# gchq/annchor

Measured on AMD Instinct MI355X. Metric: knn_graph_builds_per_s (1 / Annchor.fit() wall-clock; BASELINE: k-NN graph build time + recall@k), higher is better.
Workload: dtype int32 bit-vectors (Levenshtein) + f64 (bounds/regression/selection); 1 GPU; load_strings Levenshtein N=1600 n_anchors=15 k=25 p_work=0.12 niters=2; parallelism=one GPU

## Files before the change

### annchor_amd/csrc/common.h

```cpp
#pragma once
#include <hip/hip_runtime.h>

#include <cstdint>
#include <cstdio>
#include <cstring>
#include <string>
#include <vector>
#include <chrono>

#include "../../include/annchor_hip.h"

#define ANN_WAVE 64

struct DevBuf {
    void *p = nullptr;
    size_t cap = 0;
    bool in_arena = false;
    template <typename T> T *as() const { return reinterpret_cast<T *>(p); }
};

struct ProfEntry {
    const char *name;
    double ms = 0;
    int64_t launches = 0;
    double alg_bytes = 0;
};

struct PendingEvent {
    int entry;
    hipEvent_t a, b;
};

struct annchor_ctx {
    int device = 0;
    hipStream_t stream = nullptr;
    std::string err;
    hipDeviceProp_t prop;

    char *arena = nullptr;
    size_t arena_size = 0, arena_off = 0;

    int metric = ANNCHOR_METRIC_NONE;
    int64_t nx = 0;
    DevBuf sym, soff, slen;
    int alphabet = 0, maxlen = 0;
    bool sym_wide = false;
    int lev_gl0 = 0;
    double lev_frac0 = 0.0;
    DevBuf lev_order;
    int lev_nshort = 0;
    DevBuf lev_ap;
    DevBuf lev_ap_min;
    uint32_t lev_ap_epoch = 0;
    uint32_t lev_ap_probe_epoch = 0;
    DevBuf lev_cursors;
    int lev_cursor_epoch = 0;
    DevBuf lev_perm;
    DevBuf pts;
    int dim = 0;
    DevBuf hist, cost, supp;
    DevBuf hs_bin, hs_val, hs_cnt;
    int nbins = 0, max_support = 0;
    double cost_max = 0.0;
    int emd_epoch = 0;
    bool cost_is_metric = false;
    bool hist_integral = false;
    bool hist_fits_i16 = false;

    std::vector<unsigned char> model_cache;
    bool model_cache_valid = false;
    size_t model_cache_errs = 0;

    bool park_refine = false;
    hipEvent_t dl_ev = nullptr;

    uint32_t idle_gen_seed = 0;
    int64_t idle_gen_n = 0, idle_gen_done = 0, idle_gen_chunk = 0;

    void *comm = nullptr;
    int comm_world = 1, comm_rank = 0;
    void *comm_side = nullptr;
    hipStream_t comm_side_stream = nullptr;
    hipEvent_t comm_side_ev = nullptr, comm_main_ev = nullptr;
    bool comm_side_pending = false;
    double comm_timeout_s = 300.0;
    bool comm_aborted = false;
    void *comm_watch = nullptr;

    int na = 0, nA = 0;
    DevBuf Dt;
    DevBuf A;
    DevBuf anchorRank;
    DevBuf runmin, redval, redidx;

    DevBuf sid, cA, thr;
    int sid_nw = 1;
    DevBuf sidl, sidm;
    int sid_L = 0;
    DevBuf Kbits, Kpref;
    DevBuf deg, low, rowstart;
    DevBuf Iptr, Iidx;
    int64_t n = 0;
    DevBuf ij;
    bool have_bitmap = false;
    DevBuf colT, colM;

    DevBuf lb, ub, dad, RA, prob;
    DevBuf anc, ncm, label;
    bool have_features = false, have_RA = false;
    int64_t n_unc = -1;
    int64_t n_unc_after_features = -1;

    DevBuf spos, sy;
    DevBuf draw_J, draw_next, draw_q1;
    DevBuf sfeat, spred;
    DevBuf model;
    DevBuf ols_scratch;
    std::vector<DevBuf *> own_allocs;
    int prof_group_entry = -1;
    bool model_fitted = false;
    bool errs_on_device = false;
    int model_nb = 0;
    DevBuf dev_flags;
    bool dev_flags_clean = false;
    bool gn_err_clean = false;
    bool state_prewarmed = false;
    DevBuf sstats;
    DevBuf hs_key, hs_pos, hs_misc;
    int64_t nsamp = 0;

    DevBuf thresh;
    DevBuf cand, next;
    int64_t ncand = 0, nnext = 0;
    bool cand_marked = false;
    DevBuf gl_val, gl_pos, gl_cnt, gl_ncomp, marked, markcount;
    DevBuf gn_state;
    bool sel_prepared = false;
    int sel_k = 0, sel_nmin = 0;
    bool gn_pending = false;
    int gn_round = 0, gn_L = 0;
    DevBuf sel_hist, sel_state, blk_cnt, blk_off;
    DevBuf sel_pass_state;
    DevBuf tie_lists, tie_hist;
    const void *tie_hist_clean = nullptr;
    DevBuf sel2, sel_bufA, sel_bufB, sel_seg;
    const void *sel2_clean = nullptr;
    DevBuf errs, errptr;
    DevBuf ecdf_index;
    DevBuf cptr, cidx, cval;
    DevBuf c16, cbnd;
    DevBuf tmp0, tmp1, tmp2, tmp3;
    DevBuf scan_tmp;

    DevBuf stage_in, stage_out;

    bool prof_on = false;
    int prof_mode = 0;
    std::vector<hipEvent_t> ev_pool;
    std::vector<ProfEntry> prof;
    std::vector<PendingEvent> pending;
    hipEvent_t call_a = nullptr, call_b = nullptr;
    bool call_timed = false;
    static constexpr int PIN_SLOTS = 8;
    static constexpr size_t PIN_SLOT_BYTES = 64 * 1024;
    static constexpr size_t PIN_DL_BYTES = 1024 * 1024;
    static constexpr size_t PIN_TAIL_BYTES = 64;
    unsigned char *pin = nullptr;
    hipEvent_t pin_ev[PIN_SLOTS] = {};
    bool pin_busy[PIN_SLOTS] = {};
    int pin_next = 0;
};

const char *ann_set_err(annchor_ctx *c, const char *fmt, ...);

#define ANN_CHECK_HIP(c, expr)                                                                  \
    do {                                                                                        \
        hipError_t _e = (expr);                                                                 \
        if (_e != hipSuccess) {                                                                 \
            ann_set_err((c), "%s:%d: %s failed: %s", __FILE__, __LINE__, #expr,                 \
                        hipGetErrorString(_e));                                                 \
            return ANNCHOR_EHIP;                                                                \
        }                                                                                       \
    } while (0)

#define ANN_TRY(expr)                \
    do {                             \
        int _r = (expr);             \
        if (_r != ANNCHOR_OK) return _r; \
    } while (0)

#define ANN_REQUIRE(c, cond, code, ...)    \
    do {                                   \
        if (!(cond)) {                     \
            ann_set_err((c), __VA_ARGS__); \
            return (code);                 \
        }                                  \
    } while (0)

int ann_reserve(annchor_ctx *c, DevBuf &b, size_t bytes);
int ann_arena_init(annchor_ctx *c, int64_t nx);
int ann_prewarm_state(annchor_ctx *c);
void ann_lev_ap_probe(annchor_ctx *c);
size_t ann_sel2_table_bytes();
size_t ann_tie_hist_bytes();
size_t ann_sel_state_bytes();
int ann_h2d(annchor_ctx *c, void *dst, const void *src, size_t bytes);
hipError_t ann_sync(annchor_ctx *c, const char *where);
int ann_dev_alloc(annchor_ctx *c, void **p, size_t want, size_t *got);
void ann_dev_free(annchor_ctx *c, void *p, size_t bytes);
struct Sel2Epilogue;
int ann_kth_async(annchor_ctx *c, const double *vals, const uint8_t *flag, int64_t n, const int64_t *ks, int nk,
                  const unsigned long long **d_prefix, const int **d_unfinished, const Sel2Epilogue *epi = nullptr);
void ann_kth_async_done(annchor_ctx *c);
int ann_d2h(annchor_ctx *c, void *dst, const void *src, size_t bytes);
int ann_d2h_then(annchor_ctx *c, void *dst, const void *src, size_t bytes, int (*then)(annchor_ctx *));
int ann_d2h2(annchor_ctx *c, void *dst1, const void *src1, size_t bytes1, void *dst2, const void *src2, size_t bytes2);

int ann_prof_entry(annchor_ctx *c, const char *name);
struct ProfGroup {
    annchor_ctx *c;
    int entry = -1;
    hipEvent_t a = nullptr, b = nullptr;
    ProfGroup(annchor_ctx *ctx, const char *name);
    ~ProfGroup();
};

struct ProfScope {
    annchor_ctx *c;
    int entry = -1;
    hipEvent_t a = nullptr, b = nullptr;
    ProfScope(annchor_ctx *ctx, const char *name, double alg_bytes = 0);
    ~ProfScope();
};

static inline int ann_blocks(int64_t n, int per_block) { return (int)((n + per_block - 1) / per_block); }

__device__ __forceinline__ uint64_t ann_key_asc(double v)
{
    uint64_t u = (uint64_t)__double_as_longlong(v);
    return (u & 0x8000000000000000ull) ? ~u : (u | 0x8000000000000000ull);
}
__device__ __forceinline__ double ann_key_asc_inv(uint64_t k)
{
    uint64_t u = (k & 0x8000000000000000ull) ? (k & 0x7fffffffffffffffull) : ~k;
    return __longlong_as_double((long long)u);
}

template <typename T> __device__ __forceinline__ T ann_ldc(const T *__restrict__ p, int64_t t, int64_t n)
{
    return p[t < n ? t : n - 1];
}

#define ANN_STREAM_MIN_PAIRS (8ll << 20)
template <typename T> __device__ __forceinline__ void ann_store(T *p, T v, bool stream)
{
    if (stream) __builtin_nontemporal_store(v, p);
    else *p = v;
}
template <typename T> __device__ __forceinline__ T ann_load(const T *p, bool stream)
{
    return stream ? __builtin_nontemporal_load(p) : *p;
}

#define MAXBINS 64
struct RegModel {
    double e[MAXBINS + 1];
    double w[MAXBINS][3];
    double c[MAXBINS];
    int nb;
};
struct DeviceModel {
    RegModel reg;
    int32_t status[MAXBINS];
    int32_t err_status;
    int64_t rows[MAXBINS];
    int64_t errptr[MAXBINS + 1];
};

struct PairSource {
    const int2 *ij = nullptr;
    const int32_t *idx = nullptr;
    const int32_t *anchor = nullptr;
    int64_t n = 0;
    const double *pick_row = nullptr;
    double *pick_runmin = nullptr;
    int32_t *pick_out = nullptr;
    int pick_reset = 0;
    bool *pick_fused = nullptr;
};

#define ANN_MASK_ANCHORS 256
#define ANN_MAX_ANCHORS 1024
static_assert(ANN_MAX_ANCHORS < 0xffff, "wide sets list anchor ids as uint16, 0xffff pads");
static inline bool ann_sid_wide(int na) { return na > ANN_MASK_ANCHORS; }
__device__ __forceinline__ int sidm_common(const uint16_t *__restrict__ sidl, const uint64_t *__restrict__ sidm, int L, int na, int kw,
                                           int64_t i, int64_t w)
{
    const int lane = threadIdx.x & 63;
    int c = 0;
    for (int r = 0; r < L; ++r) {
        const int64_t e = i * L + r;
        const uint32_t pr = reinterpret_cast<const uint32_t *>(sidl)[e >> 1];
        const int a = __builtin_amdgcn_readfirstlane((int)((pr >> ((e & 1) * 16)) & 0xffffu));
        if (a >= na) continue;
        const uint64_t m = sidm[(size_t)a * kw + w];
        c += (int)((m >> lane) & 1ull);
    }
    return c;
}
template <int LC>
__device__ __forceinline__ int sidm_common_l(const uint16_t *__restrict__ sidl, const uint64_t *__restrict__ sidm, int na, int kw,
                                             int64_t i, int64_t w)
{
    const int lane = threadIdx.x & 63;
    int a[LC];
#pragma unroll
    for (int r = 0; r < LC; ++r) {
        const int64_t e = i * LC + r;
        const uint32_t pr = reinterpret_cast<const uint32_t *>(sidl)[e >> 1];
        a[r] = __builtin_amdgcn_readfirstlane((int)((pr >> ((e & 1) * 16)) & 0xffffu));
    }
    int c = 0;
#pragma unroll
    for (int r = 0; r < LC; ++r) {
        const uint64_t m = sidm[(size_t)(a[r] < na ? a[r] : 0) * kw + w];
        c += a[r] < na ? (int)((m >> lane) & 1ull) : 0;
    }
    return c;
}
template <int NW> struct Sid { uint64_t w[NW]; };
template <int NW> __device__ __forceinline__ Sid<NW> sid_ld(const uint64_t *__restrict__ sid, int64_t i)
{
    Sid<NW> s;
#pragma unroll
    for (int w = 0; w < NW; ++w) s.w[w] = sid[i * NW + w];
    return s;
}
template <int NW> __device__ __forceinline__ Sid<NW> sid_zero()
{
    Sid<NW> s;
#pragma unroll
    for (int w = 0; w < NW; ++w) s.w[w] = 0ull;
    return s;
}
template <int NW> __device__ __forceinline__ int sid_common(const Sid<NW> &a, const Sid<NW> &b)
{
    int c = 0;
#pragma unroll
    for (int w = 0; w < NW; ++w) c += __popcll(a.w[w] & b.w[w]);
    return c;
}
static inline int ann_sid_words(int na) { return na <= 64 ? 1 : na <= 128 ? 2 : na <= ANN_MASK_ANCHORS ? 4 : (na + 63) / 64; }
#define ANN_SID_DISPATCH(nw, CALL) do { if ((nw) == 1) { CALL(1); } else if ((nw) == 2) { CALL(2); } else if ((nw) == 4) { CALL(4); } \
                                        else { ANN_REQUIRE(c, false, ANNCHOR_ESTATE, "no mask kernel for %d-word anchor sets", (int)(nw)); } } while (0)

__device__ __forceinline__ void argmax_combine(double &v, int &i, double ov, int oi)
{
    if (ov > v || (ov == v && oi < i)) { v = ov; i = oi; }
}
int ann_metric_launch(annchor_ctx *c, const PairSource &src, double *d_out, double *d_RA, uint8_t *d_ncm);
int ann_lev_launch(annchor_ctx *c, const PairSource &src, double *d_out, double *d_RA, uint8_t *d_ncm);
int ann_lev_anchor_rounds(annchor_ctx *c, int32_t na, int32_t first, bool *done);
int ann_legacy_generate_upto(uint32_t seed, int64_t ndraws, int64_t upto);
static inline long long ann_now_ns()
{
    return (long long)std::chrono::duration_cast<std::chrono::nanoseconds>(std::chrono::steady_clock::now().time_since_epoch()).count();
}
int ann_legacy_scan(uint32_t seed, const int64_t *counts, const int64_t *want, int32_t nbins, uint32_t *J, const int64_t *joff,
                    void (*after_bin)(int, void *), void *user, unsigned long long *progress = nullptr);
int ann_model_prefetch_begin(annchor_ctx *c, unsigned char *at, size_t room, size_t *used);
void ann_model_prefetch_end(annchor_ctx *c, const unsigned char *at, size_t used);
int ann_euclid_launch(annchor_ctx *c, const PairSource &src, double *d_out, double *d_RA, uint8_t *d_ncm);
int ann_emd_launch(annchor_ctx *c, const PairSource &src, double *d_out, double *d_RA, uint8_t *d_ncm);

int ann_exclusive_scan_i32_to_i64(annchor_ctx *c, const int32_t *in, int64_t *out, int64_t n);
int ann_kth_smallest(annchor_ctx *c, const double *vals, const uint8_t *flag, int64_t n, const int64_t *ks,
                     int nk, double *h_out);

int ann_set_anchor_flags(annchor_ctx *c, const int64_t *hA, int nA);
int ann_dev_flags(annchor_ctx *c);
int ann_predict_merge_device(annchor_ctx *c, const RegModel *d_model, int first_iteration, int is_metric);
```

### annchor_amd/csrc/refine.hip

```cpp
#include "common.h"
#include "rowsel.h"

__global__ __launch_bounds__(ROW_THREADS) void k_comp_count(const int64_t *__restrict__ Iptr, RowSrc src, int32_t *__restrict__ cnt)
{
    __shared__ uint32_t acc;
    if (threadIdx.x == 0) acc = 0;
    __syncthreads();
    const int64_t i = row_of_block(gridDim.x), b = Iptr[i];
    const int len = (int)(Iptr[i + 1] - b);
    const RowView rv = row_view(src, i, b);
    uint32_t s = 0;
    for (int k0 = threadIdx.x; k0 < len; k0 += 4 * ROW_THREADS) {
        bool u[4];
#pragma unroll
        for (int e = 0; e < 4; ++e) u[e] = rv.unc(min(k0 + e * ROW_THREADS, len - 1));
#pragma unroll
        for (int e = 0; e < 4; ++e) s += (k0 + e * ROW_THREADS < len) && !u[e];
    }
    if (s) atomicAdd(&acc, s);
    __syncthreads();
    if (threadIdx.x == 0) cnt[i] = (int32_t)acc;
}

__global__ __launch_bounds__(ROW_THREADS) void k_comp_fill(const int64_t *__restrict__ Iptr, RowSrc src, const int2 *__restrict__ ij,
                                                          const int64_t *__restrict__ cptr,
                                                          int32_t *__restrict__ cidx, double *__restrict__ cval)
{
    __shared__ uint32_t wsum[ROW_THREADS / 64];
    const int64_t i = row_of_block(gridDim.x), b = Iptr[i];
    const int len = (int)(Iptr[i + 1] - b);
    const RowView rv = row_view(src, i, b);
    const int32_t *Iidx = src.Iidx;
    const double *RA = src.RA;
    int64_t w = cptr[i];
    for (int base = 0; base < len; base += ROW_THREADS) {
        const int k = base + threadIdx.x;
        uint32_t f = 0;
        if (k < len) f = !rv.unc(k);
        uint32_t tot;
        const uint32_t ex = row_block_scan(f, wsum, &tot);
        if (f) {
            const int32_t p = Iidx[b + k];
            const int2 q = ij[p];
            cidx[w + ex] = q.x == (int)i ? q.y : q.x;
            cval[w + ex] = RA[p];
        }
        w += tot;
        __syncthreads();
    }
}

__device__ __forceinline__ uint32_t comp_zero_bytes(uint4 v) { return 16u - (uint32_t)(__popc(v.x) + __popc(v.y) + __popc(v.z) + __popc(v.w)); }
#define COMP_ONES make_uint4(0x01010101u, 0x01010101u, 0x01010101u, 0x01010101u)

__global__ __launch_bounds__(ROW_THREADS) void k_comp_count_direct(const int64_t *__restrict__ Iptr, RowSrc src, int32_t *__restrict__ cnt)
{
    __shared__ uint32_t acc;
    if (threadIdx.x == 0) acc = 0;
    __syncthreads();
    const int64_t i = row_of_block(gridDim.x), b = Iptr[i];
    const int len = (int)(Iptr[i + 1] - b);
    const RowView rv = row_view(src, i, b);
    const int nA = min(rv.low, len);
    uint32_t s = 0;
    for (int part = 0; part < 2; ++part) {
        const uint8_t *p = part ? rv.ncm : rv.Tm;
        const int n = part ? len - nA : nA;
        const int head = min(n, (int)((16u - (uint32_t)(reinterpret_cast<uintptr_t>(p) & 15u)) & 15u));
        if ((int)threadIdx.x < head) s += p[threadIdx.x] == 0;
        const uint4 *q = reinterpret_cast<const uint4 *>(p + head);
        const int n16 = (n - head) >> 4;
        for (int t = threadIdx.x; t < n16; t += ROW_THREADS) s += comp_zero_bytes(q[t]);
        for (int k = head + (n16 << 4) + threadIdx.x; k < n; k += ROW_THREADS) s += p[k] == 0;
    }
#pragma unroll
    for (int off = 32; off > 0; off >>= 1) s += __shfl_xor(s, off);
    if ((threadIdx.x & 63) == 0 && s) atomicAdd(&acc, s);
    __syncthreads();
    if (threadIdx.x == 0) cnt[i] = (int32_t)acc;
}

__global__ __launch_bounds__(ROW_THREADS) void k_comp_fill_direct(const int64_t *__restrict__ Iptr, RowSrc src, const int2 *__restrict__ ij,
                                                                 const int64_t *__restrict__ cptr,
                                                                 int32_t *__restrict__ cidx, double *__restrict__ cval)
{
    __shared__ uint32_t wsum[ROW_THREADS / 64];
    const int64_t i = row_of_block(gridDim.x), b = Iptr[i];
    const int len = (int)(Iptr[i + 1] - b);
    const RowView rv = row_view(src, i, b);
    const int32_t *Iidx = src.Iidx + b;
    const double *RA = src.RA;
    const int nA = min(rv.low, len);
    int64_t w = cptr[i];
    auto step = [&](uint4 v, int k0) {
        const uint32_t z = comp_zero_bytes(v);
        uint32_t tot;
        uint32_t ex = row_block_scan(z, wsum, &tot);
        if (z) {
            const uint32_t wd[4] = {v.x, v.y, v.z, v.w};
#pragma unroll
            for (int e = 0; e < 16; ++e)
                if (((wd[e >> 2] >> (8 * (e & 3))) & 0xFFu) == 0u) {
                    const int32_t p = Iidx[k0 + e];
                    const int2 q = ij[p];
                    cidx[w + ex] = q.x == (int)i ? q.y : q.x;
                    cval[w + ex] = RA[p];
                    ++ex;
                }
        }
        w += tot;
        __syncthreads();
    };
    for (int part = 0; part < 2; ++part) {
        const uint8_t *p = part ? rv.ncm : rv.Tm;
        const int n = part ? len - nA : nA, kofs = part ? nA : 0;
        const int head = min(n, (int)((16u - (uint32_t)(reinterpret_cast<uintptr_t>(p) & 15u)) & 15u));
        if (head) {
            uint4 v = COMP_ONES;
            if ((int)threadIdx.x < head) v.x = 0x01010100u | p[threadIdx.x];
            step(v, kofs + (int)threadIdx.x);
        }
        const uint4 *q = reinterpret_cast<const uint4 *>(p + head);
        const int n16 = (n - head) >> 4;
        for (int t0 = 0; t0 < n16; t0 += ROW_THREADS) {
            const int t = t0 + threadIdx.x;
            step(t < n16 ? q[t] : COMP_ONES, kofs + head + (t << 4));
        }
        const int tail0 = head + (n16 << 4);
        if (tail0 < n) {
            uint4 v = COMP_ONES;
            if (tail0 + (int)threadIdx.x < n) v.x = 0x01010100u | p[tail0 + threadIdx.x];
            step(v, kofs + tail0 + (int)threadIdx.x);
        }
    }
}

#define UB_STAGE 1024
template <int G>
__global__ __launch_bounds__(256) void k_update_bounds(const int32_t *__restrict__ next, int64_t nnext,
                                                      const int2 *__restrict__ ij, const int64_t *__restrict__ cptr,
                                                      const int32_t *__restrict__ cidx, const double *__restrict__ cval,
                                                      double *__restrict__ lb, double *__restrict__ ub)
{
    constexpr int GROUPS = 256 / G, STAGE = UB_STAGE * G / 64;
    __shared__ int32_t stage[GROUPS][STAGE];
    const int lane = threadIdx.x & (G - 1), grp = threadIdx.x / G;
    const int64_t t = ((int64_t)blockIdx.x * blockDim.x + threadIdx.x) / G;
    const bool live = t < nnext;
    const int32_t p = live ? next[t] : 0;
    const int2 q = live ? ij[p] : make_int2(0, 0);
    int64_t a0 = 0, a1 = 0, b0 = 0, b1 = 0;
    if (live) { a0 = cptr[q.x]; a1 = cptr[q.x + 1]; b0 = cptr[q.y]; b1 = cptr[q.y + 1]; }
    if (a1 - a0 > b1 - b0) { int64_t x = a0; a0 = b0; b0 = x; x = a1; a1 = b1; b1 = x; }
    double nl = 0.0, nu = INFINITY;
    const int nbk = (int)(b1 - b0);
    if (nbk <= STAGE) {
        int32_t *sk = stage[grp];
        for (int e = lane; e < nbk; e += G) sk[e] = cidx[b0 + e];
        __builtin_amdgcn_fence(__ATOMIC_RELEASE, "wavefront");
        __builtin_amdgcn_wave_barrier();
        __builtin_amdgcn_fence(__ATOMIC_ACQUIRE, "wavefront");
        for (int64_t e = a0 + lane; e < a1; e += G) {
            const int32_t key = cidx[e];
            int lo = 0, hi = nbk;
            while (lo < hi) {
                const int mid = (lo + hi) >> 1;
                if (sk[mid] < key) lo = mid + 1; else hi = mid;
            }
            if (lo < nbk && sk[lo] == key) {
                const double x = cval[e], y = cval[b0 + lo];
                nu = fmin(nu, x + y);
                nl = fmax(nl, fabs(x - y));
            }
        }
    } else {
        for (int64_t e = a0 + lane; e < a1; e += G) {
            const int32_t key = cidx[e];
            int64_t lo = b0, hi = b1;
            while (lo < hi) {
                const int64_t mid = (lo + hi) >> 1;
                if (cidx[mid] < key) lo = mid + 1; else hi = mid;
            }
            if (lo < b1 && cidx[lo] == key) {
                const double x = cval[e], y = cval[lo];
                nu = fmin(nu, x + y);
                nl = fmax(nl, fabs(x - y));
            }
        }
    }
#pragma unroll
    for (int off = G / 2; off > 0; off >>= 1) {
        nu = fmin(nu, __shfl_xor(nu, off));
        nl = fmax(nl, __shfl_xor(nl, off));
    }
    if (lane == 0 && live) {
        lb[p] = fmax(nl, lb[p]);
        ub[p] = fmin(nu, ub[p]);
    }
}

#define UBB_THREADS 512
#define UBB_CHUNK 2048
#define UBB_RING 128
#define UBB_GAP 4
#define UBB_K16_WORDS 4096
__device__ __forceinline__ size_t ubb_off16(int64_t c0, int64_t j) { return (size_t)((c0 & ~(int64_t)3) + UBB_GAP * j); }

__global__ __launch_bounds__(256) void k_comp_narrow(const int64_t *__restrict__ cptr, const int32_t *__restrict__ cidx, int64_t nx,
                                                    uint16_t *__restrict__ c16, uint32_t *__restrict__ cbnd)
{
    const int lane = threadIdx.x & 63;
    const int64_t j = ((int64_t)blockIdx.x * blockDim.x + threadIdx.x) >> 6;
    if (j >= nx) return;
    const int64_t c0 = cptr[j], len = cptr[j + 1] - c0;
    uint16_t *out = c16 + ubb_off16(c0, j);
    uint32_t below = 0;
    for (int64_t e = lane; e < len; e += 64) {
        const int32_t k = cidx[c0 + e];
        out[e] = (uint16_t)k;
        below += k < 65536;
    }
#pragma unroll
    for (int off = 32; off > 0; off >>= 1) below += __shfl_xor(below, off);
    if (lane == 0) cbnd[j] = below;
}

template <bool K16, int NK, int NT, int CH>
__global__ __launch_bounds__(NT) __attribute__((amdgpu_waves_per_eu(NT == 512 ? 6 : 4, NT == 512 ? 6 : 8))) void k_update_bounds_bits(const int32_t *__restrict__ next, int64_t nnext,
                                                           const int2 *__restrict__ ij, const int64_t *__restrict__ cptr,
                                                           const int32_t *__restrict__ cidx, const uint16_t *__restrict__ c16,
                                                           const uint32_t *__restrict__ cbnd, const double *__restrict__ cval,
                                                           double *__restrict__ lb, double *__restrict__ ub, int nx)
{
    extern __shared__ __attribute__((aligned(16))) unsigned char dyn[];
    uint2 *tabw = reinterpret_cast<uint2 *>(dyn);
    const int W = (nx + 31) / 32;
    constexpr int NW = NT / 64, EPI = 64 * NK;
    static_assert(!K16 || NK % 4 == 0, "2-byte keys come four per read");
    const int TW = K16 ? UBB_K16_WORDS : W;
    const int lane = threadIdx.x & 63, wave = __builtin_amdgcn_readfirstlane((int)(threadIdx.x >> 6));
    unsigned char *after = dyn + (size_t)TW * 8;
    uint2 *ring = reinterpret_cast<uint2 *>(after) + wave * UBB_RING;
    unsigned long long *accU = reinterpret_cast<unsigned long long *>(after + NW * UBB_RING * 8) + wave * 64;
    unsigned long long *accL = reinterpret_cast<unsigned long long *>(after + NW * UBB_RING * 8 + NW * 64 * 8) + wave * 64;
    uint32_t *scan_w = reinterpret_cast<uint32_t *>(after + NW * UBB_RING * 8 + 2 * NW * 64 * 8);
    int &first_other = *reinterpret_cast<int *>(scan_w + NW);
    for (int c = threadIdx.x; c < W; c += NT) tabw[c] = make_uint2(0u, 0u);
    const int64_t t0 = (int64_t)blockIdx.x * CH, t1 = min(t0 + CH, nnext);
    int cur = -1;
    int64_t ca0 = 0, ca1 = 0;
    __syncthreads();
    for (int64_t t = t0; t < t1;) {
        const int i = ij[next[t]].x;
        if (threadIdx.x == 0) first_other = (int)(t1 - t);
        __syncthreads();
        for (int64_t tt = t + threadIdx.x; tt < t1; tt += NT)
            if (ij[next[tt]].x != i) { atomicMin(&first_other, (int)(tt - t)); break; }
        __syncthreads();
        const int seg = first_other;
        if (cur != i) {
            for (int64_t e = ca0 + threadIdx.x; e < ca1; e += NT) tabw[cidx[e] >> 5] = make_uint2(0u, 0u);
            ca0 = cptr[i]; ca1 = cptr[i + 1];
            __syncthreads();
            for (int64_t e = ca0 + threadIdx.x; e < ca1; e += NT) {
                const int cc = cidx[e];
                atomicOr(&tabw[cc >> 5].x, 1u << (cc & 31));
            }
            __syncthreads();
            const int per = (W + NT - 1) / NT, w0 = threadIdx.x * per, w1 = min(w0 + per, W);
            uint32_t mine = 0;
            for (int w = w0; w < w1; ++w) mine += (uint32_t)__popc(tabw[w].x);
            uint32_t inc = mine;
#pragma unroll
            for (int off = 1; off < 64; off <<= 1) { const uint32_t o = __shfl_up(inc, off); if (lane >= off) inc += o; }
            if (lane == 63) scan_w[wave] = inc;
            __syncthreads();
            uint32_t base = inc - mine;
            for (int w = 0; w < wave; ++w) base += scan_w[w];
            for (int w = w0; w < w1; ++w) { tabw[w].y = base; base += (uint32_t)__popc(tabw[w].x); }
            cur = i;
            __syncthreads();
        }
        for (int m0 = 0; wave + NW * m0 < seg; m0 += 64) {
            const int q = wave + NW * (m0 + lane);
            const bool have = q < seg;
            int32_t p = 0;
            int64_t c0 = 0;
            uint32_t len = 0, bd = 0;
            size_t o16 = 0;
            if (have) {
                p = next[t + q];
                const int j = ij[p].y;
                c0 = cptr[j];
                len = (uint32_t)(cptr[j + 1] - c0);
                if (K16) { bd = cbnd[j]; o16 = ubb_off16(c0, j); }
            }
            accU[lane] = 0x7FF0000000000000ull;
            accL[lane] = 0ull;
            const int npair = min(64, (seg - wave - NW * m0 + NW - 1) / NW);
            int qhead = 0, qcount = 0;
            auto drain = [&](int nf) {
                __builtin_amdgcn_fence(__ATOMIC_RELEASE, "wavefront");
                __builtin_amdgcn_wave_barrier();
                __builtin_amdgcn_fence(__ATOMIC_ACQUIRE, "wavefront");
                if (lane < nf) {
                    const uint2 e = ring[(qhead + lane) & (UBB_RING - 1)];
                    const double x = cval[ca0 + (e.x & 0xFFFFFu)], y = cval[e.y];
                    const int kk = (int)(e.x >> 20);
                    atomicMin(&accU[kk], (unsigned long long)__double_as_longlong(x + y));
                    atomicMax(&accL[kk], (unsigned long long)__double_as_longlong(fabs(x - y)));
                }
                qhead = (qhead + nf) & (UBB_RING - 1);
                qcount -= nf;
            };
            uint32_t kv[NK];
            auto request = [&](int kk, uint32_t off, uint32_t *dst) {
                const uint32_t L = (uint32_t)__builtin_amdgcn_readlane((int)len, kk);
                const uint32_t blo = (uint32_t)__builtin_amdgcn_readlane((int)(uint32_t)(K16 ? (uint64_t)o16 : (uint64_t)c0), kk);
                const uint32_t bhi = (uint32_t)__builtin_amdgcn_readlane((int)(uint32_t)((K16 ? (uint64_t)o16 : (uint64_t)c0) >> 32), kk);
                const size_t base = ((size_t)bhi << 32) | blo;
                if (K16) {
                    const uint2 *src = reinterpret_cast<const uint2 *>(c16 + base);
                    const uint32_t last4 = (max(L, 1u) - 1) >> 2;
#pragma unroll
                    for (int u = 0; u < NK / 4; ++u) {
                        const uint2 v = src[min((off >> 2) + 64 * u + lane, last4)];
                        dst[2 * u] = v.x; dst[2 * u + 1] = v.y;
                    }
                } else {
                    const int32_t *src = cidx + base;
                    const uint32_t last = max(L, 1u) - 1;
#pragma unroll
                    for (int u = 0; u < NK; ++u) dst[u] = (uint32_t)src[min(off + 64 * u + lane, last)];
                }
            };
            int kk = 0;
            uint32_t off = 0;
            if (npair > 0) request(0, 0u, kv);
            while (kk < npair) {
                const uint32_t L = (uint32_t)__builtin_amdgcn_readlane((int)len, kk);
                int nk = kk;
                uint32_t noff = off + EPI;
                if (noff >= L) { nk = kk + 1; noff = 0; }
                uint32_t nv[NK];
#pragma unroll
                for (int u = 0; u < NK; ++u) nv[u] = 0;
                if (nk < npair) request(nk, noff, nv);
                const uint32_t c0lo = (uint32_t)__builtin_amdgcn_readlane((int)(uint32_t)c0, kk);
                const uint32_t Lr = L > off ? L - off : 0u;
                uint32_t key[NK], lpos[NK];
                uint2 w[NK];
                uint32_t mask = 0;
                if (K16) {
                    const uint32_t B = (uint32_t)__builtin_amdgcn_readlane((int)bd, kk);
                    const uint32_t Br = B > off ? B - off : 0u;
                    uint32_t bitidx[NK];
#pragma unroll
                    for (int u = 0; u < NK; ++u) {
                        const uint32_t half = kv[u >> 1];
                        lpos[u] = 4u * (64u * (u >> 2) + lane) + (u & 3);
                        const uint32_t at = (((u & 1) ? half >> 18 : half >> 2) & 0x3FF8u) | (lpos[u] >= Br ? 16384u : 0u);
                        w[u] = *reinterpret_cast<const uint2 *>(dyn + at);
                        bitidx[u] = (u & 1) ? half >> 16 : half;
                        key[u] = 0;
                    }
                    uint32_t vm = 0;
#pragma unroll
                    for (int g = 0; g < NK / 4; ++g) {
                        const int nv = min(max((int)Lr - (int)(4u * (64u * g + lane)), 0), 4);
                        vm |= ((1u << nv) - 1u) << (4 * g);
                    }
#pragma unroll
                    for (int u = 0; u < NK; ++u) mask |= __builtin_amdgcn_ubfe(w[u].x, bitidx[u], 1u) << u;
                    mask &= vm;
                } else {
#pragma unroll
                    for (int u = 0; u < NK; ++u) { key[u] = kv[u]; lpos[u] = 64u * u + lane; }
#pragma unroll
                    for (int u = 0; u < NK; ++u) w[u] = tabw[key[u] >> 5];
#pragma unroll
                    for (int u = 0; u < NK; ++u) mask |= (lpos[u] < Lr ? (w[u].x >> (key[u] & 31)) & 1u : 0u) << u;
                }
                unsigned long long bal = __ballot(mask != 0);
                while (bal) {
                    if (mask) {
                        const int u = __ffs(mask) - 1;
                        mask &= mask - 1;
                        uint32_t k, lp;
                        if (K16) {
                            uint32_t half = kv[0];
#pragma unroll
                            for (int e = 1; e < NK / 2; ++e) half = (u >> 1) == e ? kv[e] : half;
                            lp = 4u * (64u * (uint32_t)(u >> 2) + lane) + (uint32_t)(u & 3);
                            const uint32_t B = (uint32_t)__builtin_amdgcn_readlane((int)bd, kk);
                            k = ((half >> ((u & 1) * 16)) & 0xFFFFu) | (off + lp >= B ? 65536u : 0u);
                        } else {
                            k = key[0]; lp = lpos[0];
#pragma unroll
                            for (int e = 1; e < NK; ++e) { k = u == e ? key[e] : k; lp = u == e ? lpos[e] : lp; }
                        }
                        const uint2 ww = tabw[k >> 5];
                        const uint32_t rank = ww.y + (uint32_t)__popc(ww.x & ((1u << (k & 31)) - 1u));
                        const int at = qcount + (int)__builtin_amdgcn_mbcnt_hi((uint32_t)(bal >> 32), __builtin_amdgcn_mbcnt_lo((uint32_t)bal, 0u));
                        ring[(qhead + at) & (UBB_RING - 1)] = make_uint2(rank | ((uint32_t)kk << 20), c0lo + off + lp);
                    }
                    qcount += __popcll(bal);
                    if (qcount >= 64) drain(64);
                    bal = __ballot(mask != 0);
                }
#pragma unroll
                for (int u = 0; u < NK; ++u) kv[u] = nv[u];
                kk = nk; off = noff;
            }
            if (qcount) drain(qcount);
            __builtin_amdgcn_fence(__ATOMIC_RELEASE, "wavefront");
            __builtin_amdgcn_wave_barrier();
            __builtin_amdgcn_fence(__ATOMIC_ACQUIRE, "wavefront");
            if (have) {
                lb[p] = fmax(__longlong_as_double((long long)accL[lane]), lb[p]);
                ub[p] = fmin(__longlong_as_double((long long)accU[lane]), ub[p]);
            }
        }
        t += seg;
        __syncthreads();
    }
}

extern "C" int annchor_update_bounds(annchor_ctx *c)
{
    if (!c) return ANNCHOR_EINVAL;
    ANN_REQUIRE(c, c->have_RA, ANNCHOR_EINVAL, "RefineApprox not initialised");
    if (c->nnext == 0) return ANNCHOR_OK;
    ANN_CHECK_HIP(c, hipSetDevice(c->device));
    const int64_t nx = c->nx;
    ANN_TRY(ann_reserve(c, c->tmp1, sizeof(int32_t) * (size_t)nx));
    ANN_TRY(ann_reserve(c, c->cptr, sizeof(int64_t) * (size_t)(nx + 1)));
    ANN_CHECK_HIP(c, hipEventRecord(c->call_a, c->stream));
    int64_t total = 0;
    RowSrc rsrc;
    ANN_TRY(ann_transpose_columns(c, &rsrc, false));
    {
        ProfScope ps(c, "computed_neighbour_csr", (double)c->n * 2 * 5.0);
        static const bool comp_generic = getenv("ANNCHOR_COMP_GENERIC") != nullptr;
        const bool comp_direct = rsrc.T != nullptr && !comp_generic;
        if (comp_direct) k_comp_count_direct<<<(int)nx, ROW_THREADS, 0, c->stream>>>(c->Iptr.as<int64_t>(), rsrc, c->tmp1.as<int32_t>());
        else
        k_comp_count<<<(int)nx, ROW_THREADS, 0, c->stream>>>(c->Iptr.as<int64_t>(), rsrc, c->tmp1.as<int32_t>());
        ANN_TRY(ann_exclusive_scan_i32_to_i64(c, c->tmp1.as<int32_t>(), c->cptr.as<int64_t>(), nx));
        if ((size_t)c->n * 2 * 12 <= ((size_t)256 << 20)) {
            total = 2 * c->n;
        } else {
            ANN_TRY(ann_d2h(c, &total, c->cptr.as<int64_t>() + nx, sizeof total));
        }
        ANN_TRY(ann_reserve(c, c->cidx, sizeof(int32_t) * (size_t)(total + 1)));
        ANN_TRY(ann_reserve(c, c->cval, sizeof(double) * (size_t)(total + 1)));
        if (comp_direct) k_comp_fill_direct<<<(int)nx, ROW_THREADS, 0, c->stream>>>(c->Iptr.as<int64_t>(), rsrc, c->ij.as<int2>(), c->cptr.as<int64_t>(),
                                                           c->cidx.as<int32_t>(), c->cval.as<double>());
        else
        k_comp_fill<<<(int)nx, ROW_THREADS, 0, c->stream>>>(c->Iptr.as<int64_t>(), rsrc, c->ij.as<int2>(), c->cptr.as<int64_t>(),
                                                           c->cidx.as<int32_t>(), c->cval.as<double>());
    }
    {
        const int64_t counted = c->n_unc >= 0 ? 2 * (c->n - c->n_unc) : total;
        const double avg = nx > 0 ? (double)counted / (double)nx : 0.0;
        const char *ube = getenv("ANNCHOR_UPDATE_BOUNDS");
        const bool long_form = ube ? strncmp(ube, "bits", 4) == 0 : avg >= 256.0;
        const bool k16 = long_form && nx <= 131072 && !(ube && strcmp(ube, "bits32") == 0);
        const int ub_waves = UBB_THREADS / 64;
        const size_t bits_bytes = (k16 ? (size_t)UBB_K16_WORDS : ((size_t)nx + 31) / 32) * 8 + (size_t)ub_waves * (UBB_RING * 8 + 2 * 64 * 8 + 4) + 16;
        const bool rows_form = long_form && bits_bytes <= 128 * 1024 && nx < (1 << 20);
        const int chunk = UBB_CHUNK;
        const double runs = (double)std::min<int64_t>(c->nnext, nx + (c->nnext + chunk - 1) / chunk);
        const double alg = rows_form ? (double)c->nnext * (avg * (k16 ? 2.0 : 4.0) + 36.0) + runs * avg * 12.0
                                     : (double)c->nnext * (2.0 * avg * 12.0 + 36.0);
        ProfScope ps(c, "update_bounds_intersect", alg);
#define UBB_ARGS c->next.as<int32_t>(), c->nnext, c->ij.as<int2>(), c->cptr.as<int64_t>(), c->cidx.as<int32_t>(), k16 ? c->c16.as<uint16_t>() : nullptr, \
                 k16 ? c->cbnd.as<uint32_t>() : nullptr, c->cval.as<double>(), c->lb.as<double>(), c->ub.as<double>(), (int)nx
        if (rows_form) {
            if (k16) {
                ANN_TRY(ann_reserve(c, c->c16, sizeof(uint16_t) * (size_t)(total + UBB_GAP * nx + 16)));
                ANN_TRY(ann_reserve(c, c->cbnd, sizeof(uint32_t) * (size_t)nx));
                k_comp_narrow<<<ann_blocks(nx * 64, 256), 256, 0, c->stream>>>(c->cptr.as<int64_t>(), c->cidx.as<int32_t>(), nx,
                                                                             c->c16.as<uint16_t>(), c->cbnd.as<uint32_t>());
            }
            if (bits_bytes > 32 * 1024) {
                if (k16) ANN_CHECK_HIP(c, hipFuncSetAttribute((const void *)k_update_bounds_bits<true, 8, UBB_THREADS, UBB_CHUNK>, hipFuncAttributeMaxDynamicSharedMemorySize, (int)bits_bytes));
                else ANN_CHECK_HIP(c, hipFuncSetAttribute((const void *)k_update_bounds_bits<false, 8, UBB_THREADS, UBB_CHUNK>, hipFuncAttributeMaxDynamicSharedMemorySize, (int)bits_bytes));
            }
            if (k16) k_update_bounds_bits<true, 8, UBB_THREADS, UBB_CHUNK><<<ann_blocks(c->nnext, UBB_CHUNK), UBB_THREADS, bits_bytes, c->stream>>>(UBB_ARGS);
            else k_update_bounds_bits<false, 8, UBB_THREADS, UBB_CHUNK><<<ann_blocks(c->nnext, UBB_CHUNK), UBB_THREADS, bits_bytes, c->stream>>>(UBB_ARGS);
        } else
#undef UBB_ARGS
        if (ube ? strcmp(ube, "pairs16") == 0 : avg < 192.0)
            k_update_bounds<16><<<ann_blocks(c->nnext * 16, 256), 256, 0, c->stream>>>(
            c->next.as<int32_t>(), c->nnext, c->ij.as<int2>(), c->cptr.as<int64_t>(), c->cidx.as<int32_t>(),
            c->cval.as<double>(), c->lb.as<double>(), c->ub.as<double>());
        else if (ube ? strcmp(ube, "pairs32") == 0 : avg < 256.0)
            k_update_bounds<32><<<ann_blocks(c->nnext * 32, 256), 256, 0, c->stream>>>(
            c->next.as<int32_t>(), c->nnext, c->ij.as<int2>(), c->cptr.as<int64_t>(), c->cidx.as<int32_t>(),
            c->cval.as<double>(), c->lb.as<double>(), c->ub.as<double>());
        else
        k_update_bounds<64><<<ann_blocks(c->nnext * 64, 256), 256, 0, c->stream>>>(
            c->next.as<int32_t>(), c->nnext, c->ij.as<int2>(), c->cptr.as<int64_t>(), c->cidx.as<int32_t>(),
            c->cval.as<double>(), c->lb.as<double>(), c->ub.as<double>());
    }
    ANN_CHECK_HIP(c, hipEventRecord(c->call_b, c->stream));
    c->call_timed = true;
    ANN_CHECK_HIP(c, hipGetLastError());
    return ANNCHOR_OK;
}


#define TR_T 64
#define TR_SUPER 16
template <bool VALUES> __global__ __launch_bounds__(256) void k_transpose_cols(const uint64_t *__restrict__ K, const uint32_t *__restrict__ pref, int kw,
                                                       const int32_t *__restrict__ low, const int64_t *__restrict__ rowstart,
                                                       const int64_t *__restrict__ Iptr, const double *__restrict__ RA,
                                                       const uint8_t *__restrict__ ncm, int64_t nx, double *__restrict__ T,
                                                       uint8_t *__restrict__ Tm)
{
    __shared__ double tv[TR_T][TR_T + 1];
    __shared__ uint8_t tm[TR_T][TR_T + 4];
    const int nb = kw;
    const int S = (nb + TR_SUPER - 1) / TR_SUPER;
    const int64_t k_in = (int64_t)blockIdx.x >> 3;
    const int64_t st = (k_in / (TR_SUPER * TR_SUPER)) * 8 + (blockIdx.x & 7);
    if (st >= (int64_t)S * (S + 1) / 2) return;
    int JB = (int)((2.0 * S + 1.0 - sqrt((2.0 * S + 1.0) * (2.0 * S + 1.0) - 8.0 * (double)st)) * 0.5);
    while ((int64_t)JB * S - (int64_t)JB * (JB - 1) / 2 > st) --JB;
    while ((int64_t)(JB + 1) * S - (int64_t)(JB + 1) * JB / 2 <= st) ++JB;
    const int IB = JB + (int)(st - ((int64_t)JB * S - (int64_t)JB * (JB - 1) / 2));
    const int w_in = (int)(k_in % (TR_SUPER * TR_SUPER));
    const int jb = JB * TR_SUPER + w_in / TR_SUPER, ib = IB * TR_SUPER + w_in % TR_SUPER;
    if (jb > ib || ib >= nb) return;
    const int lane = threadIdx.x & 63, wave = threadIdx.x >> 6;
    const int64_t i_r = (int64_t)ib * 64 + lane;
    {
        int64_t pos[16];
        bool ok[16];
#pragma unroll
        for (int q = 0; q < 16; ++q) {
            const int64_t j = min((int64_t)jb * 64 + wave * 16 + q, nx - 1);
            const uint64_t bits = K[j * kw + ib];
            ok[q] = (int64_t)jb * 64 + wave * 16 + q < nx && i_r > j && ((bits >> lane) & 1ull);
            const int64_t p = rowstart[j] + ((int64_t)pref[j * kw + ib] + __popcll(bits & ((1ull << lane) - 1ull)) - low[j]);
            pos[q] = ok[q] ? p : 0;
        }
        double v[16];
        uint8_t m[16];
#pragma unroll
        for (int q = 0; q < 16; ++q) { v[q] = VALUES ? __builtin_nontemporal_load(&RA[pos[q]]) : 0.0; m[q] = __builtin_nontemporal_load(&ncm[pos[q]]); }
#pragma unroll
        for (int q = 0; q < 16; ++q) {
            if (VALUES) tv[wave * 16 + q][lane] = ok[q] ? v[q] : 0.0;
            tm[wave * 16 + q][lane] = ok[q] ? m[q] : (uint8_t)0;
        }
    }
    __syncthreads();
    const int64_t j_w = (int64_t)jb * 64 + lane;
    uint32_t cb_lo = 0, cb_hi = 0, cd_lo = 0, cd_hi = 0;
    {
        const int64_t i = (int64_t)ib * 64 + wave * 16 + (lane & 15);
        if (i < nx) {
            const uint64_t bits = K[i * kw + jb];
            const int64_t dst0 = (Iptr[i] - rowstart[i]) + (int64_t)pref[i * kw + jb];
            cb_lo = (uint32_t)bits; cb_hi = (uint32_t)(bits >> 32);
            cd_lo = (uint32_t)dst0; cd_hi = (uint32_t)((uint64_t)dst0 >> 32);
        }
    }
#pragma unroll
    for (int q = 0; q < 16; ++q) {
        const int il = wave * 16 + q;
        const int64_t i = (int64_t)ib * 64 + il;
        const uint64_t bits = ((uint64_t)(uint32_t)__builtin_amdgcn_readlane((int)cb_hi, q) << 32) | (uint32_t)__builtin_amdgcn_readlane((int)cb_lo, q);
        if (j_w < i && ((bits >> lane) & 1ull)) {
            const int64_t dst0 = (int64_t)(((uint64_t)(uint32_t)__builtin_amdgcn_readlane((int)cd_hi, q) << 32) | (uint32_t)__builtin_amdgcn_readlane((int)cd_lo, q));
            const int64_t dst = dst0 + __popcll(bits & ((1ull << lane) - 1ull));
            if (VALUES) __builtin_nontemporal_store(tv[lane][il], &T[dst]);
            __builtin_nontemporal_store(tm[lane][il], &Tm[dst]);
        }
    }
}

#define ANN_TRANSPOSE_MIN_PAIRS (8ll << 20)
int ann_transpose_columns(annchor_ctx *c, RowSrc *src, bool with_values)
{
    src->RA = c->RA.as<double>(); src->ncm = c->ncm.as<uint8_t>(); src->Iidx = c->Iidx.as<int32_t>();
    src->T = nullptr; src->Tm = nullptr; src->rowstart = c->rowstart.as<int64_t>(); src->low = c->low.as<int32_t>();
    static const int shrink_min = getenv("ANNCHOR_ROWC_SHRINK_MIN") ? atoi(getenv("ANNCHOR_ROWC_SHRINK_MIN")) : ROWC_SHRINK_MIN;
    src->shrink_min = shrink_min;
    static const long long min_pairs = getenv("ANNCHOR_TRANSPOSE_MIN") ? atoll(getenv("ANNCHOR_TRANSPOSE_MIN")) : ANN_TRANSPOSE_MIN_PAIRS;
    if (!c->have_bitmap || c->n < min_pairs) return ANNCHOR_OK;
    ANN_TRY(ann_reserve(c, c->colT, sizeof(double) * (size_t)c->n));
    ANN_TRY(ann_reserve(c, c->colM, (size_t)c->n));
    const int kw = (int)((c->nx + 63) / 64);
    const int64_t S = (kw + TR_SUPER - 1) / TR_SUPER;
    const int64_t tiles = ((S * (S + 1) / 2 + 7) / 8) * 8 * TR_SUPER * TR_SUPER;
    if (!with_values) {
        ProfScope ps(c, "transpose_column_half_mask", (double)c->n * 2.0);
        k_transpose_cols<false><<<(unsigned)tiles, 256, 0, c->stream>>>(c->Kbits.as<uint64_t>(), c->Kpref.as<uint32_t>(), kw, c->low.as<int32_t>(),
                                                                       c->rowstart.as<int64_t>(), c->Iptr.as<int64_t>(), c->RA.as<double>(),
                                                                       c->ncm.as<uint8_t>(), c->nx, c->colT.as<double>(), c->colM.as<uint8_t>());
    } else {
        ProfScope ps(c, "transpose_column_half", (double)c->n * 18.0);
        k_transpose_cols<true><<<(unsigned)tiles, 256, 0, c->stream>>>(c->Kbits.as<uint64_t>(), c->Kpref.as<uint32_t>(), kw, c->low.as<int32_t>(),
                                                                c->rowstart.as<int64_t>(), c->Iptr.as<int64_t>(), c->RA.as<double>(),
                                                                c->ncm.as<uint8_t>(), c->nx, c->colT.as<double>(), c->colM.as<uint8_t>());
    }
    ANN_CHECK_HIP(c, hipGetLastError());
    src->T = c->colT.as<double>();
    src->Tm = c->colM.as<uint8_t>();
    return ANNCHOR_OK;
}

__global__ __launch_bounds__(ROW_THREADS) void k_get_nn(const int64_t *__restrict__ Iptr, RowSrc src,
                                                       const int2 *__restrict__ ij, int nn, int64_t *__restrict__ ngi,
                                                       double *__restrict__ ngd, int cap)
{
    __shared__ RowSelShared sh;
    __shared__ RowCand rc;
    __shared__ double wmax[ROW_THREADS / 64];
    __shared__ uint32_t cnt_lt;
    extern __shared__ __attribute__((aligned(16))) unsigned char dyn[];
    const int L = nn - 1;
    uint64_t *keys = reinterpret_cast<uint64_t *>(dyn);
    uint64_t *lkey = keys + cap;
    int32_t *lslot = reinterpret_cast<int32_t *>(lkey + L);
    const int64_t i = row_of_block(gridDim.x), b = Iptr[i];
    const int len = (int)(Iptr[i + 1] - b);
    if (threadIdx.x == 0) { ngi[i * nn] = i; ngd[i * nn] = 0.0; cnt_lt = 0; }
    const RowView rv = row_view(src, i, b);
    const int32_t *Iidx = src.Iidx;
    const double *RA = src.RA;
    __shared__ uint32_t ncomp_s, risky_s;
    if (threadIdx.x == 0) { ncomp_s = 0; risky_s = 0; }
    double mx = -INFINITY;
    uint32_t my_comp = 0, my_risky = 0;
    const int want0 = min(L, len);
    const int fast0 = want0 > 0 ? row_candidates(rc, len, want0, [&](int s) { return ann_key_asc(rv.val(s)); },
        [&](int s) { return !rv.unc(s); },
        [&](int, uint64_t kk, bool computed) {
            const double d = ann_key_asc_inv(kk);
            mx = fmax(mx, d);
            my_comp += computed;
            my_risky += !computed && !(d > 0.0);
        }) : -1;
    if (my_comp) atomicAdd(&ncomp_s, my_comp);
    if (my_risky) atomicAdd(&risky_s, my_risky);
#pragma unroll
    for (int off = 32; off > 0; off >>= 1) mx = fmax(mx, __shfl_xor(mx, off));
    if ((threadIdx.x & 63) == 0) wmax[threadIdx.x >> 6] = mx;
    __syncthreads();
    mx = fmax(fmax(wmax[0], wmax[1]), fmax(wmax[2], wmax[3]));
    if (want0 > 0 && fast0 >= want0 && (int)ncomp_s >= want0 && risky_s == 0) {
        const int fast0s = row_cand_shrink(rc, fast0, want0, src.shrink_min);
        if (fast0s >= want0) {
        for (int e = threadIdx.x; e < fast0s; e += ROW_THREADS) {
            const uint64_t ke = rc.key[e];
            const int32_t se = rc.slot[e];
            int r = 0;
            for (int o = 0; o < fast0s; ++o) { const uint64_t ko = rc.key[o]; r += (ko < ke) || (ko == ke && rc.slot[o] < se); }
            if (r < want0) {
                const int32_t p = Iidx[b + se];
                const int2 q = ij[p];
                ngi[i * nn + 1 + r] = q.x == (int)i ? q.y : q.x;
                ngd[i * nn + 1 + r] = RA[p];
            }
        }
        for (int e = want0 + threadIdx.x; e < L; e += ROW_THREADS) { ngi[i * nn + 1 + e] = 0; ngd[i * nn + 1 + e] = 0.0; }
        return;
        }
    }
    __syncthreads();
    const bool in_lds = len <= cap;
    auto key_of = [&](int s) -> uint64_t {
        const double d = rv.val(s);
        const bool u = rv.unc(s);
        return ann_key_asc(u ? d + mx : d);
    };
    const int want = min(L, len);
    {
        const int fast = want > 0 ? row_candidates(rc, len, want, key_of, [](int) { return true; },
                                                   [&](int s, uint64_t kk, bool) { if (in_lds) keys[s] = kk; }) : -1;
        const int fasts = (fast >= want && want > 0) ? row_cand_shrink(rc, fast, want, src.shrink_min) : -1;
        if (fasts >= want && want > 0) {
            for (int e = threadIdx.x; e < fasts; e += ROW_THREADS) {
                const uint64_t ke = rc.key[e];
                const int32_t se = rc.slot[e];
                int r = 0;
                for (int o = 0; o < fasts; ++o) { const uint64_t ko = rc.key[o]; r += (ko < ke) || (ko == ke && rc.slot[o] < se); }
                if (r < want) {
                    const int32_t p = Iidx[b + se];
                    const int2 q = ij[p];
                    ngi[i * nn + 1 + r] = q.x == (int)i ? q.y : q.x;
                    ngd[i * nn + 1 + r] = RA[p];
                }
            }
            for (int e = want + threadIdx.x; e < L; e += ROW_THREADS) { ngi[i * nn + 1 + e] = 0; ngd[i * nn + 1 + e] = 0.0; }
            return;
        }
        if (want <= 0 && in_lds) {  }
    }
    auto kf = [&](int s) -> uint64_t { return in_lds ? keys[s] : key_of(s); };
    if (want > 0) {
        const uint64_t t = row_kth_key(sh, len, (uint32_t)(want - 1), kf);
        for (int s = threadIdx.x; s < len; s += ROW_THREADS) {
            const uint64_t kk = kf(s);
            if (kk < t) { const uint32_t o = atomicAdd(&cnt_lt, 1u); lkey[o] = kk; lslot[o] = s; }
        }
        __syncthreads();
        uint32_t run = cnt_lt;
        for (int base = 0; base < len && run < (uint32_t)want; base += ROW_THREADS) {
            const int s = base + threadIdx.x;
            const uint32_t f = (s < len && kf(s) == t) ? 1u : 0u;
            uint32_t tot;
            const uint32_t ex = row_block_scan(f, sh.wsum, &tot);
            if (f && run + ex < (uint32_t)want) { lkey[run + ex] = t; lslot[run + ex] = s; }
            run += tot;
            __syncthreads();
        }
        __syncthreads();
        for (int e = threadIdx.x; e < want; e += ROW_THREADS) {
            const uint64_t ke = lkey[e];
            const int32_t se = lslot[e];
            int r = 0;
            for (int o = 0; o < want; ++o) r += (lkey[o] < ke) || (lkey[o] == ke && lslot[o] < se);
            const int32_t p = Iidx[b + se];
            const int2 q = ij[p];
            ngi[i * nn + 1 + r] = q.x == (int)i ? q.y : q.x;
            ngd[i * nn + 1 + r] = RA[p];
        }
    }
    for (int e = want + threadIdx.x; e < L; e += ROW_THREADS) { ngi[i * nn + 1 + e] = 0; ngd[i * nn + 1 + e] = 0.0; }
}

extern "C" int annchor_neighbor_graph(annchor_ctx *c, int32_t nn, int64_t *ng_idx, double *ng_dist)
{
    if (!c || !ng_idx || !ng_dist) return ANNCHOR_EINVAL;
    ANN_REQUIRE(c, c->have_RA, ANNCHOR_EINVAL, "RefineApprox not initialised");
    ANN_REQUIRE(c, nn >= 2 && nn <= 1024, ANNCHOR_ELIMIT, "n_neighbors=%d: 2..1024 supported", nn);
    ANN_CHECK_HIP(c, hipSetDevice(c->device));
    const size_t cells = (size_t)c->nx * nn;
    static const bool no_zc = getenv("ANNCHOR_NO_ZEROCOPY") != nullptr;
    const bool direct = c->pin && !no_zc && cells * 16 <= annchor_ctx::PIN_DL_BYTES;
    unsigned char *slot = c->pin ? c->pin + (size_t)annchor_ctx::PIN_SLOTS * annchor_ctx::PIN_SLOT_BYTES : nullptr;
    ANN_TRY(ann_reserve(c, c->stage_out, cells * 16));
    int64_t *d_i = direct ? reinterpret_cast<int64_t *>(slot) : c->stage_out.as<int64_t>();
    double *d_d = reinterpret_cast<double *>(d_i + cells);
    size_t mp_used = 0;
    unsigned char *mp_at = nullptr;
    if (direct) {
        const size_t base = (cells * 16 + 255) & ~(size_t)255;
        if (base < annchor_ctx::PIN_DL_BYTES) {
            mp_at = slot + base;
            ANN_TRY(ann_model_prefetch_begin(c, mp_at, annchor_ctx::PIN_DL_BYTES - base, &mp_used));
        }
    }
    ANN_CHECK_HIP(c, hipEventRecord(c->call_a, c->stream));
    RowSrc rsrc;
    ANN_TRY(ann_transpose_columns(c, &rsrc));
    {
        ProfScope ps(c, "row_topk_graph", (double)c->n * 2 * 13.0 + (double)cells * 16.0);
        const size_t tail = (((size_t)(nn - 1) * 12) + 15) & ~(size_t)15;
        int cap = 2;
        if (!rsrc.T) ANN_TRY(row_pick_cap(c, k_get_nn, c->nx, c->nx, tail, &cap));
        ANN_TRY(row_lds_prepare(c, k_get_nn, (size_t)cap * 8 + tail));
        k_get_nn<<<(int)c->nx, ROW_THREADS, (size_t)cap * 8 + tail, c->stream>>>(
            c->Iptr.as<int64_t>(), rsrc, c->ij.as<int2>(), nn, d_i, d_d, cap);
    }
    ANN_CHECK_HIP(c, hipEventRecord(c->call_b, c->stream));
    c->call_timed = true;
    ANN_CHECK_HIP(c, hipGetLastError());
    if (direct) {
        ANN_CHECK_HIP(c, ann_sync(c, __func__));
        ann_model_prefetch_end(c, mp_at, mp_used);
        memcpy(ng_idx, slot, cells * 8);
        memcpy(ng_dist, slot + cells * 8, cells * 8);
        return ANNCHOR_OK;
    }
    if (c->pin && cells * 16 <= annchor_ctx::PIN_DL_BYTES) {
        ANN_CHECK_HIP(c, hipMemcpyAsync(slot, d_i, cells * 16, hipMemcpyDeviceToHost, c->stream));
        ANN_CHECK_HIP(c, ann_sync(c, __func__));
        memcpy(ng_idx, slot, cells * 8);
        memcpy(ng_dist, slot + cells * 8, cells * 8);
        return ANNCHOR_OK;
    }
    ANN_TRY(ann_d2h(c, ng_idx, d_i, cells * 8));
    return ann_d2h(c, ng_dist, d_d, cells * 8);
}
```

Measured before the change: 359.4 graphs/s.

## Add bitset-word fast path for update_bounds on small point sets

For point sets of up to 2048 rows with sparse computed neighbours, each row's computed neighbours are encoded as a 32-word bitmask plus per-word prefix counts, with values placed in sorted order. Bound updates then intersect two rows by ANDing their bitmasks across 8 lanes and use popcount to locate the matching values. This replaces the count, scan, fill and intersect pipeline with two kernels and removes the scan and its host-side total. It adds a second code path that only works when nx is at most 2048, and it assumes each row holds at most 2048 entries, since longer rows are truncated.

After: 343.2 graphs/s. 0.955x the previous value.

```diff
diff --git a/annchor_amd/csrc/common.h b/annchor_amd/csrc/common.h
--- a/annchor_amd/csrc/common.h
+++ b/annchor_amd/csrc/common.h
@@ -149,6 +149,7 @@
     DevBuf ecdf_index;
     DevBuf cptr, cidx, cval;
     DevBuf c16, cbnd;
+    DevBuf cwords;
     DevBuf tmp0, tmp1, tmp2, tmp3;
     DevBuf scan_tmp;
 
diff --git a/annchor_amd/csrc/refine.hip b/annchor_amd/csrc/refine.hip
--- a/annchor_amd/csrc/refine.hip
+++ b/annchor_amd/csrc/refine.hip
@@ -426,6 +426,125 @@
     }
 }
 
+#define UBW_WORDS 32
+#define UBW_MAX_POINTS (64 * UBW_WORDS)
+#define UBW_LANES 8
+#define UBW_PER (UBW_WORDS / UBW_LANES)
+#define UBW_BATCH 4
+static_assert(UBW_PER == 4, "a lane reads its words as two 16-byte loads and its counts as one 8-byte load");
+
+__global__ __launch_bounds__(ROW_THREADS) void k_comp_words(const int64_t *__restrict__ Iptr, RowSrc src, const int2 *__restrict__ ij,
+                                                           unsigned long long *__restrict__ bits, uint16_t *__restrict__ pre,
+                                                           double *__restrict__ cval)
+{
+    __shared__ unsigned long long wb[UBW_WORDS];
+    __shared__ uint32_t wp[UBW_WORDS];
+    const int64_t i = row_of_block(gridDim.x), b = Iptr[i];
+    const int len = min((int)(Iptr[i + 1] - b), UBW_MAX_POINTS);
+    const RowView rv = row_view(src, i, b);
+    const int32_t *Iidx = src.Iidx + b;
+    const double *RA = src.RA;
+    if (threadIdx.x < UBW_WORDS) wb[threadIdx.x] = 0ull;
+    __syncthreads();
+    constexpr int PER = UBW_MAX_POINTS / ROW_THREADS;
+    bool comp[PER];
+    int32_t other[PER];
+    double val[PER];
+#pragma unroll
+    for (int e = 0; e < PER; ++e) {
+        const int k = threadIdx.x + e * ROW_THREADS;
+        comp[e] = k < len && !rv.unc(min(k, len - 1));
+    }
+#pragma unroll
+    for (int e = 0; e < PER; ++e) {
+        other[e] = 0; val[e] = 0.0;
+        if (comp[e]) {
+            const int32_t p = Iidx[threadIdx.x + e * ROW_THREADS];
+            const int2 q = ij[p];
+            other[e] = q.x == (int)i ? q.y : q.x;
+            val[e] = RA[p];
+            atomicOr(&wb[other[e] >> 6], 1ull << (other[e] & 63));
+        }
+    }
+    __syncthreads();
+    if (threadIdx.x < UBW_WORDS) {
+        const unsigned long long w = wb[threadIdx.x];
+        const uint32_t cnt = (uint32_t)__popcll(w);
+        uint32_t inc = cnt;
+#pragma unroll
+        for (int off = 1; off < UBW_WORDS; off <<= 1) { const uint32_t o = __shfl_up(inc, off); if ((int)threadIdx.x >= off) inc += o; }
+        wp[threadIdx.x] = inc - cnt;
+        bits[i * UBW_WORDS + threadIdx.x] = w;
+        pre[i * UBW_WORDS + threadIdx.x] = (uint16_t)(inc - cnt);
+    }
+    __syncthreads();
+#pragma unroll
+    for (int e = 0; e < PER; ++e)
+        if (comp[e]) {
+            const int w = other[e] >> 6;
+            cval[b + wp[w] + (uint32_t)__popcll(wb[w] & ((1ull << (other[e] & 63)) - 1ull))] = val[e];
+        }
+}
+
+__global__ __launch_bounds__(256) void k_update_bounds_words(const int32_t *__restrict__ next, int64_t nnext, const int2 *__restrict__ ij,
+                                                            const int64_t *__restrict__ Iptr, const unsigned long long *__restrict__ bits,
+                                                            const uint16_t *__restrict__ pre, const double *__restrict__ cval,
+                                                            double *__restrict__ lb, double *__restrict__ ub)
+{
+    const int lane = threadIdx.x & (UBW_LANES - 1);
+    const int64_t t = ((int64_t)blockIdx.x * blockDim.x + threadIdx.x) / UBW_LANES;
+    const bool live = t < nnext;
+    const int32_t p = live ? next[t] : 0;
+    const int2 q = live ? ij[p] : make_int2(0, 0);
+    const size_t oi = (size_t)q.x * UBW_WORDS + UBW_PER * lane, oj = (size_t)q.y * UBW_WORDS + UBW_PER * lane;
+    const ulonglong2 ai0 = *reinterpret_cast<const ulonglong2 *>(bits + oi), ai1 = *reinterpret_cast<const ulonglong2 *>(bits + oi + 2);
+    const ulonglong2 aj0 = *reinterpret_cast<const ulonglong2 *>(bits + oj), aj1 = *reinterpret_cast<const ulonglong2 *>(bits + oj + 2);
+    const uint2 ci = *reinterpret_cast<const uint2 *>(pre + oi), cj = *reinterpret_cast<const uint2 *>(pre + oj);
+    const int64_t bi = Iptr[q.x], bj = Iptr[q.y];
+    const unsigned long long A[UBW_PER] = {ai0.x, ai0.y, ai1.x, ai1.y}, B[UBW_PER] = {aj0.x, aj0.y, aj1.x, aj1.y};
+    const uint32_t PI[UBW_PER] = {ci.x & 0xFFFFu, ci.x >> 16, ci.y & 0xFFFFu, ci.y >> 16};
+    const uint32_t PJ[UBW_PER] = {cj.x & 0xFFFFu, cj.x >> 16, cj.y & 0xFFFFu, cj.y >> 16};
+    unsigned long long M[UBW_PER];
+#pragma unroll
+    for (int w = 0; w < UBW_PER; ++w) M[w] = live ? A[w] & B[w] : 0ull;
+    double nl = 0.0, nu = INFINITY;
+    while (M[0] | M[1] | M[2] | M[3]) {
+        int64_t ei[UBW_BATCH], ej[UBW_BATCH];
+#pragma unroll
+        for (int u = 0; u < UBW_BATCH; ++u) {
+            const int w = M[0] ? 0 : M[1] ? 1 : M[2] ? 2 : 3;
+            const unsigned long long mw = w == 0 ? M[0] : w == 1 ? M[1] : w == 2 ? M[2] : M[3];
+            const unsigned long long aw = w == 0 ? A[0] : w == 1 ? A[1] : w == 2 ? A[2] : A[3];
+            const unsigned long long bw = w == 0 ? B[0] : w == 1 ? B[1] : w == 2 ? B[2] : B[3];
+            const uint32_t pi = w == 0 ? PI[0] : w == 1 ? PI[1] : w == 2 ? PI[2] : PI[3];
+            const uint32_t pj = w == 0 ? PJ[0] : w == 1 ? PJ[1] : w == 2 ? PJ[2] : PJ[3];
+            const unsigned long long below = (mw & (0ull - mw)) - 1ull;
+            const bool ok = mw != 0ull;
+            ei[u] = ok ? bi + pi + __popcll(aw & below) : (u ? ei[0] : bi);
+            ej[u] = ok ? bj + pj + __popcll(bw & below) : (u ? ej[0] : bj);
+#pragma unroll
+            for (int k = 0; k < UBW_PER; ++k) M[k] = k == w ? M[k] & (M[k] - 1ull) : M[k];
+        }
+        double x[UBW_BATCH], y[UBW_BATCH];
+#pragma unroll
+        for (int u = 0; u < UBW_BATCH; ++u) { x[u] = cval[ei[u]]; y[u] = cval[ej[u]]; }
+#pragma unroll
+        for (int u = 0; u < UBW_BATCH; ++u) {
+            nu = fmin(nu, x[u] + y[u]);
+            nl = fmax(nl, fabs(x[u] - y[u]));
+        }
+    }
+#pragma unroll
+    for (int off = UBW_LANES / 2; off > 0; off >>= 1) {
+        nu = fmin(nu, __shfl_xor(nu, off));
+        nl = fmax(nl, __shfl_xor(nl, off));
+    }
+    if (lane == 0 && live) {
+        lb[p] = fmax(nl, lb[p]);
+        ub[p] = fmin(nu, ub[p]);
+    }
+}
+
 extern "C" int annchor_update_bounds(annchor_ctx *c)
 {
     if (!c) return ANNCHOR_EINVAL;
@@ -433,6 +552,31 @@
     if (c->nnext == 0) return ANNCHOR_OK;
     ANN_CHECK_HIP(c, hipSetDevice(c->device));
     const int64_t nx = c->nx;
+    const char *ube = getenv("ANNCHOR_UPDATE_BOUNDS");
+    const double avg_short = c->n_unc >= 0 ? 2.0 * (double)(c->n - c->n_unc) / (double)nx : 2.0 * (double)c->n / (double)nx;
+    if (nx <= UBW_MAX_POINTS && (ube ? strcmp(ube, "words") == 0 : avg_short < 256.0)) {
+        ANN_TRY(ann_reserve(c, c->cwords, (size_t)nx * UBW_WORDS * (sizeof(unsigned long long) + sizeof(uint16_t))));
+        ANN_TRY(ann_reserve(c, c->cval, sizeof(double) * (size_t)(2 * c->n + 1)));
+        unsigned long long *bits = c->cwords.as<unsigned long long>();
+        uint16_t *pre = reinterpret_cast<uint16_t *>(bits + (size_t)nx * UBW_WORDS);
+        ANN_CHECK_HIP(c, hipEventRecord(c->call_a, c->stream));
+        RowSrc rsrc;
+        ANN_TRY(ann_transpose_columns(c, &rsrc, false));
+        {
+            ProfScope ps(c, "computed_neighbour_csr", (double)c->n * 2 * 5.0);
+            k_comp_words<<<(int)nx, ROW_THREADS, 0, c->stream>>>(c->Iptr.as<int64_t>(), rsrc, c->ij.as<int2>(), bits, pre, c->cval.as<double>());
+        }
+        {
+            ProfScope ps(c, "update_bounds_intersect", (double)c->nnext * (2.0 * UBW_WORDS * 10.0 + 36.0));
+            k_update_bounds_words<<<ann_blocks(c->nnext * UBW_LANES, 256), 256, 0, c->stream>>>(
+                c->next.as<int32_t>(), c->nnext, c->ij.as<int2>(), c->Iptr.as<int64_t>(), bits, pre, c->cval.as<double>(),
+                c->lb.as<double>(), c->ub.as<double>());
+        }
+        ANN_CHECK_HIP(c, hipEventRecord(c->call_b, c->stream));
+        c->call_timed = true;
+        ANN_CHECK_HIP(c, hipGetLastError());
+        return ANNCHOR_OK;
+    }
     ANN_TRY(ann_reserve(c, c->tmp1, sizeof(int32_t) * (size_t)nx));
     ANN_TRY(ann_reserve(c, c->cptr, sizeof(int64_t) * (size_t)(nx + 1)));
     ANN_CHECK_HIP(c, hipEventRecord(c->call_a, c->stream));
@@ -463,7 +607,6 @@
     {
         const int64_t counted = c->n_unc >= 0 ? 2 * (c->n - c->n_unc) : total;
         const double avg = nx > 0 ? (double)counted / (double)nx : 0.0;
-        const char *ube = getenv("ANNCHOR_UPDATE_BOUNDS");
         const bool long_form = ube ? strncmp(ube, "bits", 4) == 0 : avg >= 256.0;
         const bool k16 = long_form && nx <= 131072 && !(ube && strcmp(ube, "bits32") == 0);
         const int ub_waves = UBB_THREADS / 64;
```
